# UVA-Computer-Vision-Lab/LabelAny3D

Hardware: AMD Instinct MI355X
Metric: fitted 3D boxes/sec @640x480 (higher is better)
Workload: dtype f64

## Files before the change

labelany3d_amd/csrc/la3d_device.hpp:

```cpp
#pragma once
#ifndef LA3D_NT
#define LA3D_NT 512
#endif
#include <hip/hip_runtime.h>
#include <mutex>
#include <utility>
#include <vector>
#include <math.h>
#include <stdint.h>
#include <stdio.h>
#include <string.h>

#include "la3d.h"

namespace la3d {


constexpr int NT = LA3D_NT;
constexpr int NWAVE = NT / 64;
constexpr int NTP = 256;
constexpr int NWAVEP = NTP / 64;
constexpr double PI_2 = 1.57079632679489661923;
typedef unsigned int u32x4 __attribute__((ext_vector_type(4)));

// ... 489 lines not shown
    for (int i = tid; i < nwords; i += NTH) {
      const unsigned w = src[i];
      bits[i] = w;
      n += __popc(w);
    }
  }
  if ((HW & 31) && tid == owner) {
    const unsigned w = bits[nwords - 1], keep = w & ((1u << (HW & 31)) - 1u);
    bits[nwords - 1] = keep;
    n -= __popc(w ^ keep);
  }
  return n;
}

constexpr int GEO_D = 20;

struct alignas(16) Shared {
  double part[NWAVE][7];
  double M[9];
  double Rg[9];
  double cyaw, syaw;
  int cnt[NWAVE];
  int nmask[NWAVE];
  unsigned scan[NWAVE];
  int n_valid;
  int st;
  int bad_ground;
  int redo;
  double gap;
  int nm;
  int order_inst;
  unsigned qhead;
  int sep_bad;
  unsigned qpad[2];
#ifdef LA3D_TIMELINE
  double* tl;
#endif
};
#ifndef LA3D_TIMELINE
static_assert(sizeof(Shared) == 752, "include/la3d.h (convex-hull yaw, rule 2) and oracle/campaigns/hull.py state this size");
#endif
__device__ inline void write_no_box(const FitParams& p, int inst, int status, double n_valid, double nm) {
  if (p.aux) {
    double* a = p.aux + (long long)inst * LA3D_AUX;
    a[0] = NAN; a[1] = n_valid; a[2] = nm; a[3] = NAN;
  }
  p.status[inst] = status;
  write_nan_box(p.out + (long long)inst * LA3D_REC);
  if (p.proj) { for (int j = 0; j < 8; ++j) p.proj[(long long)inst * 8 + j] = NAN; }
}
__device__ inline void write_no_box_axis(const Shared* sh, const FitParams& p, int inst) {
  if (p.aux) {
    double* a = p.aux + (long long)inst * LA3D_AUX;
    a[0] = atan2(sh->syaw, sh->cyaw); a[1] = (double)sh->n_valid; a[2] = (double)sh->nm; a[3] = sh->gap;
  }
  p.status[inst] = sh->st;
  write_nan_box(p.out + (long long)inst * LA3D_REC);
  if (p.proj) { for (int j = 0; j < 8; ++j) p.proj[(long long)inst * 8 + j] = NAN; }
}

#ifdef LA3D_TIMELINE
#define LA3D_SUBSTAMP(sh, k) do { if (threadIdx.x == 0 && (sh)->tl) (sh)->tl[k] = (double)wall_clock64(); } while (0)
#else
#define LA3D_SUBSTAMP(sh, k) do { } while (0)
#endif

__host__ __device__ inline int mask_bit_bytes(int HW) { return ((((HW + 15) / 16 + 1) / 2) * 4 + 15) & ~15; }
// ... 120 lines not shown
      } else {
        double x = d * r0, z = d * r2;
        if (PIV) { x = fma(d, r0, m ? -px0 : 0.0); z = fma(d, r2, m ? -pz0 : 0.0); }
        s[0] += x; s[1] += z;
        s[2] = fma(x, x, s[2]); s[3] = fma(x, z, s[3]); s[4] = fma(z, z, s[4]);
      }
      if (CHK) *n -= m;
    } else {
      const unsigned bits = db[k] | ~(unsigned)m;
      const double d = (double)__uint_as_float(bits);
      const double x = d * r0, z = d * r2;
      s[0] = dmin(s[0], x); s[1] = dmax(s[1], x);
      s[4] = dmin(s[4], z); s[5] = dmax(s[5], z);
      if (SPEC) {
        fk[k] = __uint_as_float(bits);
      } else {
        const double y = d * r1;
        s[2] = dmin(s[2], y); s[3] = dmax(s[3], y);
        r1 += a10;
      }
    }
    r0 += a00;
    if (!(SPEC && PASS == 0)) r2 += a20;
  }
  if (SPEC && PASS == 1) {
    const double dlo = (double)min_f32_raw(min3_f32(fk[0], fk[1], fk[2]), fk[3]);
    const double dhi = (double)max_f32_raw(max3_f32(fk[0], fk[1], fk[2]), fk[3]);
    const double ya = dlo * r1, yb = dhi * r1;
    s[2] = dmin(s[2], dmin(ya, yb)); s[3] = dmax(s[3], dmax(ya, yb));
  }
}


template <int NTH>
__device__ inline void column_xor_scan(unsigned* bits, int H, int ntx, unsigned* scratch, int scratch_words, int tid) {
  int RB = NTH / ntx;
  if (RB > scratch_words / ntx) RB = scratch_words / ntx;
  if (RB < 1) RB = 1;
  const int RPB = (H + RB - 1) / RB;
  const int items = ntx * RB;
  if (RB > 1) {
    for (int it = tid; it < items; it += NTH) {
      const int blk = it / ntx, cw = it - blk * ntx;
      const int r1 = min(blk * RPB + RPB, H);
      unsigned x = 0;
      for (int r = blk * RPB; r < r1; ++r) x ^= bits[r * ntx + cw];
      scratch[it] = x;
    }
    __syncthreads();
  }
  for (int it = tid; it < items; it += NTH) {
    const int blk = it / ntx, cw = it - blk * ntx;
    const int r1 = min(blk * RPB + RPB, H);
    unsigned carry = 0;
    for (int b2 = 0; b2 < blk; ++b2) carry ^= scratch[b2 * ntx + cw];
    for (int r = blk * RPB; r < r1; ++r) {
      carry ^= bits[r * ntx + cw];
      bits[r * ntx + cw] = carry;
    }
  }
}

template <int NTH>
__device__ inline int rle_to_bits(const int* __restrict__ counts, int nr, unsigned* bits, int nwords, int H, int W,
                                  unsigned* wtot, int tid, unsigned* scratch = nullptr, int scratch_words = 0, int frame_w = 0) {
  const int lane = tid & 63, wave = tid >> 6;
  constexpr int NW = NTH / 64;
  const int HW = H * (frame_w > 0 && frame_w < W ? frame_w : W);
  const float rcpH = 1.0f / (float)H;
  for (int i = tid; i < nwords; i += NTH) bits[i] = 0;
  unsigned carry = 0;
  int nm = 0;
  const bool toggles = (W & 31) == 0 && scratch != nullptr && scratch_words >= 2 * (W >> 5);
  for (int c0 = 0; c0 < nr; c0 += NTH) {
    const int j = c0 + tid;
    unsigned len = 0;
    if (j < nr) { const int v = counts[j]; len = v > 0 ? (unsigned)v : 0u; }
    unsigned incl = len;
#pragma unroll
    for (int o = 1; o < 64; o <<= 1) {
      const unsigned t = __shfl_up(incl, o);
      if (lane >= o) incl += t;
    }
    __syncthreads();
    if (lane == 63) wtot[wave] = incl;
    __syncthreads();
    unsigned base = carry, total = 0;
    for (int w = 0; w < NW; ++w) { if (w < wave) base += wtot[w]; total += wtot[w]; }
    const unsigned start = base + incl - len;
    unsigned L = 0;
    if ((j & 1) && len > 0 && start < (unsigned)HW) L = min(len, (unsigned)HW - start);
    nm += (int)L;
    carry += total;
    unsigned long long todo = __ballot(L != 0);
    if (toggles) {
      const int ntx = W >> 5;
      unsigned long long wrap = 0;
      unsigned c_first = 0, c_last = 0;
      if (L != 0) {
        unsigned col0, row0, cole, rowe;
        pix_uv(start, H, rcpH, &row0, &col0);
        pix_uv(start + L, H, rcpH, &rowe, &cole);
        atomicXor(&bits[row0 * ntx + (col0 >> 5)], 1u << (col0 & 31));
        if (rowe != 0) atomicXor(&bits[rowe * ntx + (cole >> 5)], 1u << (cole & 31));
        c_first = col0 + 1;
        c_last = rowe != 0 ? cole : cole - 1;
      }
      wrap = __ballot(L != 0 && c_last >= c_first);
      while (wrap) {
        const int src = __ffsll((long long)wrap) - 1;
        wrap &= wrap - 1;
        const unsigned cf = (unsigned)__builtin_amdgcn_readlane((int)c_first, src);
        const unsigned cl = (unsigned)__builtin_amdgcn_readlane((int)c_last, src);
        for (unsigned cw = (cf >> 5) + lane; cw <= (cl >> 5); cw += 64) {
          const unsigned lo = cw == (cf >> 5) ? (cf & 31u) : 0u, hi = cw == (cl >> 5) ? (cl & 31u) : 31u;
          atomicXor(&bits[cw], (0xffffffffu >> (31u - hi)) & (0xffffffffu << lo));
        }
      }
      todo = 0;
    }
    while (todo) {
      const int src = __ffsll((long long)todo) - 1;
      todo &= todo - 1;
      const unsigned S = __shfl(start, src), Lr = __shfl(L, src);
      unsigned col0, row0;
      pix_uv(S, H, rcpH, &row0, &col0);
      if (row0 + Lr <= (unsigned)H) {
        const unsigned base = row0 * (unsigned)W + col0;
        for (unsigned q = lane; q < Lr; q += 64) {
          const unsigned idx = base + q * (unsigned)W;
          atomicOr(&bits[idx >> 5], 1u << (idx & 31));
        }
      } else {
        for (unsigned q = lane; q < Lr; q += 64) {
          unsigned col, row;
          pix_uv(S + q, H, rcpH, &row, &col);
          const unsigned idx = row * (unsigned)W + col;
          atomicOr(&bits[idx >> 5], 1u << (idx & 31));
        }
      }
    }
    if (carry >= (unsigned)HW) break;
  }
  __syncthreads();
  if (toggles) {
    column_xor_scan<NTH>(bits, H, W >> 5, scratch, scratch_words, tid);
    __syncthreads();
  }
  return nm;
}

inline int check_launch(const char* what) {
  const hipError_t e = hipGetLastError();
  if (e != hipSuccess) {
    snprintf(g_err, sizeof(g_err), "%s: %s", what, hipGetErrorString(e));
    return LA3D_ERR_HIP;
  }
  return LA3D_SUCCESS;
}

inline void allow_big_lds(const void* fn, int bytes = 160 * 1024) {
  static std::mutex mu;
  static std::vector<std::pair<const void*, int>> done;
  int dev = 0;
  if (hipGetDevice(&dev) != hipSuccess) (void)hipGetLastError();
  std::lock_guard<std::mutex> g(mu);
  for (const auto& d : done)
    if (d.first == fn && d.second == dev) return;
  if (hipFuncSetAttribute(fn, hipFuncAttributeMaxDynamicSharedMemorySize, bytes) != hipSuccess) (void)hipGetLastError();
  done.emplace_back(fn, dev);
}

constexpr int CULL_MIN = 224;
constexpr int MAX_MASK_LDS = 128 * 1024;

}
```

labelany3d_amd/csrc/la3d_instance.hip:

```cpp
#include <algorithm>
#include <atomic>
#include <chrono>
#include <cstdint>
#include <cstddef>
#include <cstring>
#include <mutex>
#include <type_traits>
#include <utility>
#include <vector>

#include "la3d_device.hpp"
#include "la3d_poly.hpp"
#include "la3d_engines.hpp"
#include "la3d_walks.hpp"
#include "la3d_stages.hpp"
#include "la3d_instance_phases.hpp"
#include "la3d_hull.hpp"

#ifndef LA3D_INSTANCE_DT
#define LA3D_INSTANCE_DT 0
#endif
#if LA3D_INSTANCE_DT == 0
using DepthT = float;
using KParams = la3d::FitParams;
// ... 170 lines not shown
    while (wall_clock64() - t0 < w) __builtin_amdgcn_s_sleep(32);
  }
  int my_draw = 0;
  if (SAMPLE && tid < LA3D_NSAMPLE) my_draw = p.sample_idx[(long long)inst * LA3D_NSAMPLE + tid];
  int nmask = 0;
  if constexpr (LDSMASK) nmask = mask_to_bits<VEC, SRC, FRAMES>(p, p_call, inst, mpl, bits, sh, list, TILED ? p.list_cap / 2 : 0, tid, wave, lane);
  __syncthreads();
  LA3D_STAMP(1);
  const int inst_p = __builtin_amdgcn_readfirstlane(sh->order_inst);
  if constexpr (FRAMES) frame_geometry<false, SAMPLE>(p_frame, p_call, p.image_index[inst_p]);
  const int tid_plain = tid;
#define tid (REBUILD_TID ? tid_here(wave, lane) : tid_plain)
  if (SRC != 0 && LDSMASK && p.filter_boundary >= 0) {
    if (!filter_keep<SRC>(p, sh, bits, inst_p, tid)) return;
  }
  double Mg[9];
#pragma unroll
  for (int i = 0; i < 9; ++i) Mg[i] = uniform_f64(sh->M[i]);
  LA3D_STAMP(13);

  bool sampled = false;
  int ntot = 0;
  if (SAMPLE) {
    const int wsum = wave_sum_i(nmask);
    if (lane == 0) sh->nmask[wave] = wsum;
    __syncthreads();
    for (int w = 0; w < NWAVE; ++w) ntot += sh->nmask[w];
    sampled = HULL || ntot > LA3D_NSAMPLE;
  }

  constexpr bool LK = TILED && !SAMPLE;
  const bool sep_cam = LK && (HULL || !p.sep_off) && Mg[1] == 0.0 && Mg[3] == 0.0 && Mg[6] == 0.0 && Mg[7] == 0.0 && Mg[8] == 1.0;
  TileList tiles;
  if (TILED && !sampled) {
    if constexpr (FRAMES) frame_rcp_ntx(p_frame);
    tiles = build_tile_list<LK>(p, sh, bits, list, sep_cam, tid, wave, lane);
    LA3D_STAMP(15);
    __syncthreads();
  }
  const int nactive = tiles.nactive, nfull = tiles.nfull, compact = tiles.compact;
  const bool sep = tiles.sep;

  if constexpr (HULL && LK) {
    hull_full_mask(sh, p, inst_p, dpl, bits, list, nactive, sep, Mg, nmask, wave, lane, cv);
    return;
  }

  if constexpr (LK) {
    if (sep) {
      LA3D_STAMP(2);
      unsigned* col = bits + nactive * 8;
      double sacc[5] = {0, 0, 0, 0, 0}, yx[2] = {INFINITY, -INFINITY};
      unsigned unsafe = 0u;
      if (p.H & 7) sweep_sep<true>(p, dpl, bits, list, nactive, Mg, col, wave, lane, sacc, yx, &unsafe, 0, nfull, cv);
      else sweep_sep<false>(p, dpl, bits, list, nactive, Mg, col, wave, lane, sacc, yx, &unsafe, 0, nfull, cv);
      if (__ballot(unsafe >= 0x7f800000u) != 0ull && lane == 0) sh->sep_bad = 1;
      const double ylo_w = uniform_f64(wave_min(yx[0])), yhi_w = uniform_f64(wave_max(yx[1]));
      LA3D_STAMP(3);
      stage_moments_to_axis(sh, p, inst_p, sacc, nmask, nmask, tid, wave, lane, true);
      LA3D_STAMP(4);
      if (!(sh->redo || sh->sep_bad)) {
        if (sh->st != LA3D_BOX_OK) return;
        double N0[3], N2[3], ext[6];
        yaw_rows(sh, Mg, N0, N2);
        sep_col_extents(col, p.W, N0, N2, tid, ext);
        ext[2] = ylo_w; ext[3] = yhi_w;
        LA3D_STAMP(5);
        if constexpr (FRAMES) frame_proj(p_frame, p_call, inst_p);
        stage_extents_to_box(sh, p, inst_p, ext, tid, wave, lane);
        stage_status_aux(sh, p, inst_p, tid);
        LA3D_STAMP(6);
        return;
      }
      __syncthreads();
    }
  }

  bool cull = false;
  int rng_words = 0;
  if constexpr (LK) {
    if (compact) {
      rng_words = cull_rng_words(nactive);
      cull = nactive >= p.cull_min && nactive <= CULL_MAXT;
      if (!cull) {
        unsigned short* surv = reinterpret_cast<unsigned short*>(bits + nactive * 8);
#pragma clang loop vectorize(disable) interleave(disable) unroll(disable)
        for (int t = tid; t < nactive; t += NT) surv[t] = (unsigned short)t;
      }
    }
  }

  LA3D_STAMP(2);
  double acc[5] = {0, 0, 0, 0, 0};
  int cnt = 0;
  double px = 0, py = 0, pz = 0;
  bool pok = false;

  if (SAMPLE) {
// ... 248 lines not shown
```

labelany3d_amd/csrc/la3d_instance_phases.hpp:

```cpp
#pragma once
#include "la3d_device.hpp"
#include "la3d_poly.hpp"
#include "la3d_hull.hpp"

using namespace la3d;

namespace {
template <bool VEC, int SRC, bool FRAMES>
__device__ inline int mask_to_bits(const FitParams& p, const FitParams& call, int inst, const unsigned char* mpl, unsigned* bits, Shared* sh,
                                   void* stage, int stage_words, int tid, int wave, int lane) {
  const int HW = p.HW;
  int nmask = 0;
  if constexpr (SRC == 1) {
    const long long o0 = p.rle_offsets[inst];
    nmask = rle_to_bits<NT>(p.rle_counts + o0, (int)(p.rle_offsets[inst + 1] - o0), bits, p.nwords, p.H, p.W, sh->scan, tid,
                            static_cast<unsigned*>(stage), stage_words, p.frame_w);
  } else if constexpr (SRC == 2) {
    nmask = poly_to_bits<NT>(p.poly_xy, p.poly_ring_off, p.poly_inst_rings[inst], p.poly_inst_rings[inst + 1],
                             static_cast<PolySide*>(stage), sh->scan, bits, p.nwords, p.H, p.W, tid, p.frame_w);
  } else if constexpr (SRC == 3) {
    if constexpr (FRAMES) nmask = bits_plane_to_lds<NT>(p.mask_bits + frame_bits_offset(call, inst), bits, p.nwords, HW, 1, tid);
    else nmask = bits_plane_to_lds<NT>(p.mask_bits + (long long)inst * p.bits_plane_stride, bits, p.nwords, HW, p.bits_vec, tid);
  } else {
    unsigned short* b16 = reinterpret_cast<unsigned short*>(bits);
    const int ngroups = (HW + 15) >> 4;
    if (VEC) {
      const u32x4* m4 = reinterpret_cast<const u32x4*>(mpl);
      constexpr int P0U = 4;
      unsigned seen = 0;
#pragma unroll P0U
      for (int g = tid; g < ngroups; g += NT) {
        const u32x4 w = __builtin_nontemporal_load(m4 + g);
        const unsigned lo = __builtin_amdgcn_udot4(w.y, 0x80402010u, __builtin_amdgcn_udot4(w.x, 0x08040201u, 0u, false), false);
        const unsigned hi = __builtin_amdgcn_udot4(w.w, 0x80402010u, __builtin_amdgcn_udot4(w.z, 0x08040201u, 0u, false), false);
        const unsigned pat = lo | (hi << 8);
        seen |= (w.x | w.y) | (w.z | w.w);
        b16[g] = (unsigned short)pat;
        nmask += __popc(pat);
      }
      const unsigned long long odd = __ballot((seen & 0xfefefefeu) != 0);
      if (lane == 0) sh->scan[wave] = odd != 0 ? 1u : 0u;
      __syncthreads();
      unsigned general = 0;
#pragma unroll
      for (int w = 0; w < NWAVE; ++w) general |= sh->scan[w];
      if (general) {
        nmask = 0;
#pragma unroll 4
        for (int g = tid; g < ngroups; g += NT) {
          const u32x4 w = m4[g];
          const unsigned pat = nz16(w.x, w.y, w.z, w.w);
          b16[g] = (unsigned short)pat;
// ... 1 lines not shown
        }
      }
    } else {
      for (int g = tid; g < ngroups; g += NT) {
        unsigned pat = 0;
        for (int k = 0; k < 16; ++k) {
          const int i = g * 16 + k;
          if (i < HW && mpl[i]) pat |= 1u << k;
        }
        b16[g] = (unsigned short)pat;
        nmask += __popc(pat);
      }
    }
    if ((ngroups & 1) && tid == 0) b16[ngroups] = 0;
  }
  return nmask;
}

template <int SRC>
__device__ inline bool filter_keep(const FitParams& p, Shared* sh, const unsigned* bits, int inst, int tid) {
  int st4[4];
  bits_filter_stats<NT>(bits, p.H, p.frame_w, p.filter_boundary, reinterpret_cast<int*>(sh->part), tid, st4, p.W);
  if (p.filter_stats && tid < 4) (p.filter_stats + (long long)inst * 4)[tid] = st4[tid];
  const int height = SRC == 1 ? st4[1] : (SRC == 3 && !p.bits_span) ? st4[1] : st4[2];
  const bool keep = 16 * height > p.H && st4[3] < p.filter_max_edge && st4[0] >= p.filter_min_area;
  if (!keep && tid == 0) write_no_box(p, inst, LA3D_BOX_FILTERED, 0.0, (double)st4[0]);
  return keep;
}

struct TileList {
  int nactive = 0, nfull = 0, compact = 0;
  bool sep = false;
};

template <bool WHOLE_ROWS, bool LK>
__device__ inline void classify_tiles(const FitParams& p, const unsigned* bits, int tbeg, int tend, int lane, unsigned long long* bal,
                                      unsigned (*wrd)[8], int* wcount, int* fcount, unsigned* fl) {
#pragma unroll
  for (int k = 0; k < 4; ++k) {
    const int t = tbeg + k * 64 + lane;
    unsigned any = 0, all = 0xffffffffu;
    if (t < tend) {
      const int ty = (int)(((float)t + 0.5f) * p.rcp_ntx), tx = t - ty * p.ntx;
      const int rmax = p.H - 1 - ty * 8;
      const unsigned* bw = bits + (ty * 8) * p.ntx + tx;
#pragma unroll
      for (int rr = 0; rr < 8; ++rr) {
        const unsigned w = bw[(WHOLE_ROWS ? rr : min(rr, rmax)) * p.ntx];
        any |= w;
        if constexpr (LK) { wrd[k][rr] = (WHOLE_ROWS || rr <= rmax) ? w : 0u; all &= wrd[k][rr]; }
      }
    }
    bal[k] = __ballot(any != 0);
    *wcount += __popcll(bal[k]);
    if constexpr (LK) {
      const bool f = t < tend && all == 0xffffffffu;
      *fcount += __popcll(__ballot(f));
      *fl |= (f ? 1u : 0u) << k;
    }
  }
}

template <bool LK>
__device__ inline TileList build_tile_list(const FitParams& p, Shared* sh, unsigned* bits, unsigned short* list, bool sep_cam, int tid, int wave, int lane) {
  TileList tl;
  const int ntiles = p.ntx * p.nty, per = p.tiles_per_wave;
// ... 51 lines not shown
  } else {
#pragma unroll 1
    for (int pass = 0; pass < 2; ++pass) {
      int wcount = 0;
      for (int t0 = tbeg; t0 < tend; t0 += 64) {
        const int t = t0 + lane;
        unsigned any = 0, packed = 0;
        if (t < tend) {
          const int ty = t / p.ntx, tx = t - ty * p.ntx;
          const int rows = min(8, p.H - ty * 8);
          const unsigned* bw = bits + (ty * 8) * p.ntx + tx;
          for (int rr = 0; rr < rows; ++rr) any |= bw[rr * p.ntx];
          packed = ((unsigned)ty << 8) | (unsigned)tx;
        }
        const unsigned long long bal = __ballot(any != 0);
        if (pass == 1 && any) list[base + wcount + __popcll(bal & ((1ull << lane) - 1ull))] = (unsigned short)packed;
        wcount += __popcll(bal);
      }
      if (pass == 0) {
        if (lane == 0) sh->scan[wave] = (unsigned)wcount;
        __syncthreads();
        for (int w = 0; w < NWAVE; ++w) {
          const int c = (int)sh->scan[w];
          if (w < wave) base += c;
          tl.nactive += c;
        }
        if (tl.nactive > p.list_cap) { tl.nactive = -1; break; }
      }
    }
  }
  return tl;
}

template <bool HULL, bool FRAMES, typename DepthT>
__device__ inline void sample_pick(const FitParams& p, Shared* sh, const unsigned* bits, unsigned* prefix, const DepthT* __restrict__ dpl,
                                          const DepthCvt<DepthT> cv, const double* Mg, int ntot, int my_draw, int tid, int wave, int lane,
                                          double* acc, int* cnt, double* ppx, double* ppy, double* ppz, bool* ppok) {
  const int nblk = (p.nwords + 31) >> 5;
  unsigned run0 = 0;
  for (int b0 = 0; b0 < nblk; b0 += NT) {
    const int blk = b0 + tid;
    unsigned local = 0;
    if (blk < nblk) {
      const int w0 = blk << 5, wn = min(32, p.nwords - w0);
      if (wn == 32) {
        const uint4* q = reinterpret_cast<const uint4*>(bits + w0);
#pragma unroll
        for (int i = 0; i < 8; ++i) { const uint4 v = q[i]; local += __popc(v.x) + __popc(v.y) + __popc(v.z) + __popc(v.w); }
      } else {
        for (int i = 0; i < wn; ++i) local += __popc(bits[w0 + i]);
      }
    }
    unsigned incl = local;
#pragma unroll
    for (int o = 1; o < 64; o <<= 1) {
      const unsigned t = __shfl_up(incl, o);
      if (lane >= o) incl += t;
    }
    if (lane == 63) sh->scan[wave] = incl;
    __syncthreads();
    unsigned base = run0, tot = 0;
    for (int w = 0; w < NWAVE; ++w) { const unsigned c = sh->scan[w]; if (w < wave) base += c; tot += c; }
    if (blk < nblk) prefix[blk] = base + incl - local;
    run0 += tot;
    __syncthreads();
  }
// ... 64 lines not shown
```

labelany3d_amd/csrc/la3d_poly.hpp:

```cpp
#pragma once
#include "la3d_device.hpp"

namespace la3d {

struct alignas(8) PolyEdge {
  int y0, y1;
  long long x, dx;
};

struct alignas(8) PolySide {
  PolyEdge e;
  int sx, sy, ex, ey;
};

constexpr int POLY_XY_SHIFT = 16;
constexpr int POLY_CHUNK = 32;
constexpr int POLY_MAX_JOINT = 8;
constexpr int POLY_META_INTS = 48;
constexpr int POLY_STAGE_BYTES = POLY_CHUNK * (int)sizeof(PolySide) + POLY_META_INTS * 4;
#ifndef LA3D_POLY_KEEP
#define LA3D_POLY_KEEP 4
#endif
constexpr int POLY_KEEP = LA3D_POLY_KEEP;

// ... 78 lines not shown

__device__ inline void poly_set_bit(unsigned* bits, int W, int x, int y) {
  const unsigned i = (unsigned)y * (unsigned)W + (unsigned)x;
  atomicOr(&bits[i >> 5], 1u << (i & 31));
}

__device__ inline void poly_draw(const PolySide& s, int W, unsigned* bits, int lane) {
  if (s.sx > s.ex) return;
  const int dx = s.ex - s.sx, dy = s.ey - s.sy;
  const int ady = dy < 0 ? -dy : dy, sgn = dy < 0 ? -1 : 1;
  if (ady > dx) {
    for (int i = lane; i <= ady; i += 64) {
      const int k = (int)((2u * (unsigned)i * (unsigned)dx + (unsigned)ady - 1u) / (2u * (unsigned)ady));
      poly_set_bit(bits, W, s.sx + k, s.sy + sgn * i);
    }
  } else {
    for (int i = lane; i <= dx; i += 64) {
      const int k = dx ? (int)((2u * (unsigned)i * (unsigned)ady + (unsigned)dx - 1u) / (2u * (unsigned)dx)) : 0;
      poly_set_bit(bits, W, s.sx + i, s.sy + sgn * k);
    }
  }
}

__device__ inline void poly_fill_span(unsigned* bits, int W, int y, int x1, int x2) {
  const unsigned i1 = (unsigned)y * (unsigned)W + (unsigned)x1, i2 = (unsigned)y * (unsigned)W + (unsigned)x2;
  const unsigned w1 = i1 >> 5, w2 = i2 >> 5;
  const unsigned m1 = 0xffffffffu << (i1 & 31), m2 = 0xffffffffu >> (31 - (i2 & 31));
  if (w1 == w2) { atomicOr(&bits[w1], m1 & m2); return; }
  atomicOr(&bits[w1], m1);
  for (unsigned w = w1 + 1; w < w2; ++w) atomicOr(&bits[w], 0xffffffffu);
  atomicOr(&bits[w2], m2);
}

template <int NTH>
__device__ __forceinline__ void poly_ring_fast(const int* __restrict__ xy, long long p0, int n, const int* rb, int nrb, PolySide* stage,
                                      int* box, unsigned* bits, int H, int W, int tid, int clipW) {
  const int lane = tid & 63, wave = tid >> 6;
  constexpr int NW = NTH / 64;
  const int ntxw = W >> 5;
  if (tid == 0) { box[0] = H; box[1] = 0; box[2] = ntxw; box[3] = 0; }
  for (int pass = 0; pass < 2; ++pass) {
    for (int c0 = 0; c0 < n; c0 += POLY_CHUNK) {
      const int m = min(POLY_CHUNK, n - c0);
      if (pass == 0 || n > POLY_CHUNK) {
        __syncthreads();
        if (tid < m) {
          const int i = c0 + tid;
          int lo = 0, hi = n;
          for (int j = 0; j < nrb; ++j)
            if (i >= rb[j] && i < rb[j + 1]) { lo = rb[j]; hi = rb[j + 1]; }
          const int ip = (i == lo) ? hi - 1 : i - 1;
          const PolySide sd = poly_side(xy[2 * (p0 + ip)], xy[2 * (p0 + ip) + 1], xy[2 * (p0 + i)], xy[2 * (p0 + i) + 1], clipW, H);
          stage[tid] = sd;
          if (pass == 0 && sd.e.y0 < sd.e.y1) {
            const int ya = max(sd.e.y0, 0), yb = min(sd.e.y1, H);
            if (ya < yb) {
              const long long fa = (sd.e.x + (long long)(ya - sd.e.y0) * sd.e.dx) >> POLY_XY_SHIFT;
              const long long fb = (sd.e.x + (long long)(yb - 1 - sd.e.y0) * sd.e.dx) >> POLY_XY_SHIFT;
              const long long lo = (fa < fb ? fa : fb) + 1, hi = (fa < fb ? fb : fa) + 1;
              atomicMin(&box[0], ya); atomicMax(&box[1], yb);
              if (lo < W) atomicMin(&box[2], (int)((lo < 0 ? 0 : lo) >> 5));
              atomicMax(&box[3], (int)((hi >= W ? W - 1 : (hi < 0 ? 0 : hi)) >> 5));
            }
          }
        }
      }
      __syncthreads();
      for (int j = wave; j < m; j += NW) {
        if (pass == 1) poly_draw(stage[j], W, bits, lane);
        const int y0 = stage[j].e.y0, y1 = stage[j].e.y1;
        if (y0 >= y1) continue;
        const long long ex = stage[j].e.x, edx = stage[j].e.dx;
        const int yb = min(y1, H);
        for (int y = max(y0, 0) + lane; y < yb; y += 64) {
          const long long f = (ex + (long long)(y - y0) * edx) >> POLY_XY_SHIFT;
          if (pass == 0) {
            const long long pos = f < -1 ? 0 : f + 1;
            if (pos < W) atomicXor(&bits[y * ntxw + (int)(pos >> 5)], 1u << ((int)pos & 31));
          } else if (f >= 0 && f < W) {
            atomicOr(&bits[y * ntxw + (int)(f >> 5)], 1u << ((int)f & 31));
          }
        }
      }
    }
    if (pass == 0) {
// ... 63 lines not shown
                }
              }
            }
          }
        }
      }
      const int npairs = min(found, POLY_KEEP) >> 1;
#pragma unroll
      for (int k = 0; k < POLY_KEEP / 2; ++k) {
        if (k < npairs) {
          const long long c1 = cx[2 * k] >> POLY_XY_SHIFT, c2 = cx[2 * k + 1] >> POLY_XY_SHIFT;
          if (c1 < W && c2 >= 0) poly_fill_span(bits, W, y, (int)(c1 < 0 ? 0 : c1), (int)(c2 >= W ? W - 1 : c2));
        }
      }
      const bool more = found > POLY_KEEP;
      if (more) { lastx = cx[POLY_KEEP - 1]; lasti = ci[POLY_KEEP - 1]; }
      first = false;
      const unsigned long long any = __ballot(more);
      __syncthreads();
      if (lane == 0) flags[wave] = any != 0 ? 1u : 0u;
      __syncthreads();
      unsigned again = 0;
#pragma unroll
      for (int w = 0; w < NW; ++w) again |= flags[w];
      if (!again) break;
    }
  }
}

__device__ inline long long poly_uniform(long long v) {
  return ((long long)__builtin_amdgcn_readfirstlane((int)(v >> 32)) << 32) | (unsigned)__builtin_amdgcn_readfirstlane((int)v);
}

template <int NTH>
__device__ __forceinline__ int poly_to_bits(const int* __restrict__ xy, const long long* __restrict__ ring_off, long long r0, long long r1,
                                   PolySide* stage, unsigned* flags, unsigned* bits, int nwords, int H, int W, int tid, int clipW = 0) {
  if (clipW <= 0 || clipW > W) clipW = W;
  r0 = poly_uniform(r0); r1 = poly_uniform(r1);
  for (int i = tid; i < nwords; i += NTH) bits[i] = 0;
  int* meta = reinterpret_cast<int*>(stage + POLY_CHUNK);
  const int nr = (int)(r1 - r0);
  long long r = r0;
  if (nr >= 1 && (W & 31) == 0) {
    int joint = 1;
    if (nr >= 2 && nr <= POLY_MAX_JOINT) {
      const int lane = tid & 63, wave = tid >> 6;
      const long long pf = ring_off[r0];
      for (int j = wave; j < nr; j += NTH / 64) {
        const long long a = ring_off[r0 + j], b = ring_off[r0 + j + 1];
        int x0 = 0x7fffffff, x1 = -0x7fffffff - 1, y0 = 0x7fffffff, y1 = -0x7fffffff - 1;
        for (long long q = a + lane; q < b; q += 64) {
          const int x = xy[2 * q], y = xy[2 * q + 1];
          x0 = min(x0, x); x1 = max(x1, x); y0 = min(y0, y); y1 = max(y1, y);
        }
        x0 = wave_min_i(x0); x1 = wave_max_i(x1); y0 = wave_min_i(y0); y1 = wave_max_i(y1);
        if (lane == 0) { meta[9 + 4 * j] = x0; meta[10 + 4 * j] = x1; meta[11 + 4 * j] = y0; meta[12 + 4 * j] = y1; meta[j] = (int)(a - pf); }
      }
      if (tid == 0) meta[nr] = (int)(ring_off[r1] - pf);
      __syncthreads();
      if (tid == 0) {
        int ok = 1;
        for (int i = 0; i < nr; ++i)
          for (int j = i + 1; j < nr; ++j) {
            const bool apart = meta[10 + 4 * i] < meta[9 + 4 * j] || meta[10 + 4 * j] < meta[9 + 4 * i] ||
                               meta[12 + 4 * i] < meta[11 + 4 * j] || meta[12 + 4 * j] < meta[11 + 4 * i];
            if (!apart) ok = 0;
          }
        meta[41] = ok;
      }
      __syncthreads();
      if (meta[41]) joint = nr;
    }
    const long long p0 = poly_uniform(ring_off[r0]);
    const int n = __builtin_amdgcn_readfirstlane((int)(ring_off[r0 + joint] - p0));
    if (joint == 1) {
      if (tid == 0) { meta[0] = 0; meta[1] = n; }
      __syncthreads();
    }
    poly_ring_fast<NTH>(xy, p0, n, meta, joint, stage, reinterpret_cast<int*>(flags), bits, H, W, tid, clipW);
    r = r0 + joint;
  }
  for (; r < r1; ++r) {
    const long long p0 = poly_uniform(ring_off[r]);
    const int n = __builtin_amdgcn_readfirstlane((int)(ring_off[r + 1] - p0));
    poly_ring_general<NTH>(xy, p0, n, stage, flags, bits, H, W, tid, clipW);
  }
  __syncthreads();
  if (clipW < W) {
    const int ntxw = W >> 5, wq = clipW >> 5, per = ntxw - wq;
    const unsigned keep = (1u << (clipW & 31)) - 1u;
    for (int i = tid; i < H * per; i += NTH) {
      const int row = i / per, k = i - row * per;
      unsigned* w = bits + row * ntxw + wq + k;
      *w = k == 0 ? (*w & keep) : 0u;
    }
    __syncthreads();
  }
  int nm = 0;
  for (int i = tid; i < nwords; i += NTH) nm += __popc(bits[i]);
  return nm;
}

__device__ inline void bits_stats_256(const unsigned* bits, int H, int W, int boundary, int* rowcnt, int* red, int tid, int* out4) {
  const int lane = tid & 63, wave = tid >> 6;
  const int bc = min(boundary, W), br = min(boundary, H);
  int area = 0, edge = 0;
  for (int r = tid; r < H; r += 256) {
    int cnt = 0, e = 0;
    const unsigned base = (unsigned)r * (unsigned)W;
    for (int c0 = 0; c0 < W; c0 += 32) {
      const unsigned i = base + c0, wi = i >> 5, sh = i & 31;
      unsigned w = bits[wi] >> sh;
      if (sh && c0 + (32 - (int)sh) < W) w |= bits[wi + 1] << (32 - sh);
      const int valid = min(32, W - c0);
      if (valid < 32) w &= (1u << valid) - 1u;
      cnt += __popc(w);
      const int nlo = min(max(bc - c0, 0), 32), fhi = min(max(W - bc - c0, 0), 32);
      e += __popc(nlo >= 32 ? w : (w & ((1u << nlo) - 1u))) + __popc(fhi >= 32 ? 0u : (w & ~((1u << fhi) - 1u)));
    }
    rowcnt[r] = cnt;
    area += cnt;
    edge += e + cnt * ((r < br ? 1 : 0) + (r >= H - br ? 1 : 0));
  }
  area = wave_sum_i(area);
  edge = wave_sum_i(edge);
  if (lane == 0) { red[12 + wave] = area; red[16 + wave] = edge; }
  __syncthreads();
  int rows = 0, first = H, last = -1;
  for (int r = tid; r < H; r += 256)
    if (rowcnt[r] != 0) { rows += 1; first = min(first, r); last = max(last, r); }
  rows = wave_sum_i(rows);
// ... 13 lines not shown
```

labelany3d_amd/csrc/la3d_walks.hpp:

```cpp
#pragma once
#include "la3d_device.hpp"

using namespace la3d;

namespace {
template <bool VEC, bool LDSMASK, int PASS, bool PIV = false, typename DT = float>
__device__ inline void sweep(const FitParams& p, const DT* __restrict__ dpl, const unsigned char* __restrict__ mpl,
                             const unsigned* bits, const double* A0, const double* A1, const double* A2,
                             int wave, int lane, double* acc, int* cnt, int* nmask, const double* pivot = nullptr,
                             const DepthCvt<DT> cv = {}) {
  double px0 = 0, pz0 = 0;
  if constexpr (PIV) { px0 = pivot[0]; pz0 = pivot[1]; }
  const int HW = p.HW, W = p.W;
  const int nquads = (HW + 3) >> 2;
  const int nchunks = (nquads + 63) >> 6;
  const double a00 = A0[0], a01 = A0[1], a02 = A0[2];
  const double a20 = A2[0], a21 = A2[1], a22 = A2[2];
  double a10 = 0, a11 = 0, a12 = 0;
  if (PASS == 1) { a10 = A1[0]; a11 = A1[1]; a12 = A1[2]; }
  double s0 = acc[0], s1 = acc[1], s2 = acc[2], s3 = acc[3], s4 = acc[4];
  double xlo = acc[0], xhi = acc[1], ylo = acc[2], yhi = acc[3], zlo = acc[4], zhi = acc[5];
  int n = *cnt, nm = *nmask;
  for (int ch = wave; ch < nchunks; ch += NWAVE) {
    const int q = ch * 64 + lane;
// ... 405 lines not shown
        ry += a11;
      }
      const double r0 = fma(a00, (double)(tx * 32 + c), a02);
      const double t1 = r0 * c1, t2 = r0 * c2;
      s0 += t1; s1 += c1; s2 = fma(r0, t2, s2); s3 += t2; s4 += c2;
      bad = max(bad, cmax);
      atomicMin(colq + tx * 32, cmin);
      atomicMax(colq + tx * 32 + p.W, cmax);
      __builtin_amdgcn_sched_barrier(0);
    }
  }
}

template <bool EDGE = false, typename DT = float>
__device__ inline void sweep_sep(const FitParams& p, const DT* __restrict__ dpl, const unsigned* bits,
                                 const unsigned short* list, int nactive, const double* Mg, unsigned* col, int wave, int lane,
                                 double* acc, double* yext, unsigned* unsafe, int row0 = 0, int nfull = 0, const DepthCvt<DT> cv = {}) {
  const int c = lane & 31, h4 = (lane >> 5) * 4;
  const double a00 = Mg[0], a02 = Mg[2], a11 = Mg[4], a12 = Mg[5];
  unsigned loff[4];
#pragma unroll
  for (int k = 0; k < 4; ++k) loff[k] = (unsigned)((h4 + k) * p.W + c) * (unsigned)sizeof(DT);
  unsigned* colq = col + c;
  double s0 = acc[0], s1 = acc[1], s2 = acc[2], s3 = acc[3], s4 = acc[4];
  double ylo = yext[0], yhi = yext[1];
  unsigned bad = *unsafe;
  if (nfull > 0) sep_steps<EDGE, true, DT>(p, dpl, bits, list, 0, nfull, a00, a02, a11, a12, colq, wave, c, h4, loff, row0, s0, s1, s2, s3, s4, ylo, yhi, bad, cv);
  sep_steps<EDGE, false, DT>(p, dpl, bits, list, nfull, nactive, a00, a02, a11, a12, colq, wave, c, h4, loff, row0, s0, s1, s2, s3, s4, ylo, yhi, bad, cv);
  acc[0] = s0; acc[1] = s1; acc[2] = s2; acc[3] = s3; acc[4] = s4;
  yext[0] = ylo; yext[1] = yhi;
  *unsafe = bad;
}

__device__ inline void sep_col_extents(const unsigned* col, int W, const double* N0, const double* N2, int tid, double* ext) {
  double xlo = INFINITY, xhi = -INFINITY, zlo = INFINITY, zhi = -INFINITY;
  for (int u = tid; u < W; u += NT) {
    const unsigned lo = col[u], hi = col[W + u];
    if (lo <= hi) {
      const double dlo = (double)__uint_as_float(lo), dhi = (double)__uint_as_float(hi), ud = (double)u;
      const double q0 = fma(N0[0], ud, N0[2]), q2 = fma(N2[0], ud, N2[2]);
      const double xa = dlo * q0, xb = dhi * q0, za = dlo * q2, zb = dhi * q2;
      xlo = fmin(xlo, fmin(xa, xb)); xhi = fmax(xhi, fmax(xa, xb));
      zlo = fmin(zlo, fmin(za, zb)); zhi = fmax(zhi, fmax(za, zb));
    }
  }
  ext[0] = xlo; ext[1] = xhi; ext[4] = zlo; ext[5] = zhi;
}

}
```

Measured before the change: 11.72 million.

## Track mask bounding box during decode and restrict scan, tiling, and extents to it

RLE and polygon decoders now record a coarse bounding box of the mask (in 32-column words and 8-row tiles) and pack it into shared memory. The column XOR scan, popcount, tile classification/list build, and column-extent reduction then iterate only over that box instead of the full frame. This targets work spent on empty regions of small masks. In exchange it adds atomics for box tracking, a fallback to the full frame when the box logic does not apply, and edge-case risk in box clipping.

```diff
diff --git a/labelany3d_amd/csrc/la3d_device.hpp b/labelany3d_amd/csrc/la3d_device.hpp
--- a/labelany3d_amd/csrc/la3d_device.hpp
+++ b/labelany3d_amd/csrc/la3d_device.hpp
@@ -545,7 +545,8 @@
   int order_inst;
   unsigned qhead;
   int sep_bad;
-  unsigned qpad[2];
+  unsigned mbox;
+  unsigned qpad;
 #ifdef LA3D_TIMELINE
   double* tl;
 #endif
@@ -732,6 +733,49 @@
 }
 
 
+constexpr unsigned MASK_BOX_EMPTY = 0x00010001u;
+__device__ inline unsigned mask_box_pack(int c0, int c1, int r0, int r1) {
+  if (c1 < c0 || r1 < r0) return MASK_BOX_EMPTY;
+  return (unsigned)min(c0 >> 5, 255) | ((unsigned)min(c1 >> 5, 255) << 8) | ((unsigned)min(r0 >> 3, 255) << 16) | ((unsigned)min(r1 >> 3, 255) << 24);
+}
+__device__ inline unsigned mask_box_whole(int H, int W) { return mask_box_pack(0, W - 1, 0, H - 1); }
+
+template <int NTH>
+__device__ inline void column_xor_scan(unsigned* bits, int H, int ntx, unsigned* scratch, int scratch_words, int tid);
+
+template <int NTH>
+__device__ inline void column_xor_scan_box(unsigned* bits, int H, int ntx, int cw0, int ncw, int r0, int nrows, unsigned* scratch,
+                                           int scratch_words, int tid) {
+  if (ncw > NTH || ncw > scratch_words) {
+    column_xor_scan<NTH>(bits, H, ntx, scratch, scratch_words, tid);
+    return;
+  }
+  const float rcp = 1.0f / (float)ncw;
+  int RB = (int)(((float)min(NTH, scratch_words) + 0.5f) * rcp);
+  RB = max(min(min(RB, 24), nrows), 1);
+  const int RPB = (int)(((float)(nrows + RB - 1) + 0.5f) * (1.0f / (float)RB));
+  const int items = ncw * RB;
+  const int blk = (int)(((float)tid + 0.5f) * rcp), c = tid - blk * ncw;
+  const int ra = r0 + blk * RPB, rb = min(ra + RPB, r0 + nrows);
+  unsigned* bw = bits + cw0 + c;
+  if (RB > 1) {
+    if (tid < items) {
+      unsigned x = 0;
+      for (int r = ra; r < rb; ++r) x ^= bw[r * ntx];
+      scratch[tid] = x;
+    }
+    __syncthreads();
+  }
+  if (tid < items) {
+    unsigned carry = 0;
+    for (int b2 = 0; b2 < blk; ++b2) carry ^= scratch[b2 * ncw + c];
+    for (int r = ra; r < rb; ++r) {
+      carry ^= bw[r * ntx];
+      bw[r * ntx] = carry;
+    }
+  }
+}
+
 template <int NTH>
 __device__ inline void column_xor_scan(unsigned* bits, int H, int ntx, unsigned* scratch, int scratch_words, int tid) {
   int RB = NTH / ntx;
@@ -761,9 +805,10 @@
   }
 }
 
-template <int NTH>
+template <int NTH, bool BOX = false>
 __device__ inline int rle_to_bits(const int* __restrict__ counts, int nr, unsigned* bits, int nwords, int H, int W,
-                                  unsigned* wtot, int tid, unsigned* scratch = nullptr, int scratch_words = 0, int frame_w = 0) {
+                                  unsigned* wtot, int tid, unsigned* scratch = nullptr, int scratch_words = 0, int frame_w = 0,
+                                  unsigned* box_out = nullptr) {
   const int lane = tid & 63, wave = tid >> 6;
   constexpr int NW = NTH / 64;
   const int HW = H * (frame_w > 0 && frame_w < W ? frame_w : W);
@@ -772,6 +817,12 @@
   unsigned carry = 0;
   int nm = 0;
   const bool toggles = (W & 31) == 0 && scratch != nullptr && scratch_words >= 2 * (W >> 5);
+  const bool boxed = BOX && toggles && scratch_words >= 2 * (W >> 5) + 4;
+  int* gbox = reinterpret_cast<int*>(scratch + (boxed ? scratch_words - 4 : 0));
+  int bc0 = 0x7fffffff, bc1 = -1, br0 = 0x7fffffff, br1 = -1;
+  if constexpr (BOX) {
+    if (boxed && tid == 0) { gbox[0] = 0x7fffffff; gbox[1] = -1; gbox[2] = 0x7fffffff; gbox[3] = -1; }
+  }
   for (int c0 = 0; c0 < nr; c0 += NTH) {
     const int j = c0 + tid;
     unsigned len = 0;
@@ -805,6 +856,12 @@
         if (rowe != 0) atomicXor(&bits[rowe * ntx + (cole >> 5)], 1u << (cole & 31));
         c_first = col0 + 1;
         c_last = rowe != 0 ? cole : cole - 1;
+        if constexpr (BOX) {
+          bc0 = min(bc0, (int)col0); bc1 = max(bc1, (int)c_last);
+          const bool one_col = c_last == col0;
+          br0 = one_col ? min(br0, (int)row0) : 0;
+          br1 = one_col ? max(br1, rowe != 0 ? (int)rowe - 1 : H - 1) : H - 1;
+        }
       }
       wrap = __ballot(L != 0 && c_last >= c_first);
       while (wrap) {
@@ -842,7 +899,24 @@
     }
     if (carry >= (unsigned)HW) break;
   }
+  if constexpr (BOX) {
+    if (boxed) {
+      bc0 = wave_min_i(bc0); bc1 = wave_max_i(bc1); br0 = wave_min_i(br0); br1 = wave_max_i(br1);
+      if (lane == 0 && bc1 >= 0) { atomicMin(&gbox[0], bc0); atomicMax(&gbox[1], bc1); atomicMin(&gbox[2], br0); atomicMax(&gbox[3], br1); }
+    }
+  }
   __syncthreads();
+  if constexpr (BOX) {
+    if (boxed) {
+      const int c0 = __builtin_amdgcn_readfirstlane(gbox[0]), c1 = __builtin_amdgcn_readfirstlane(gbox[1]);
+      const int r0 = __builtin_amdgcn_readfirstlane(gbox[2]), r1 = __builtin_amdgcn_readfirstlane(gbox[3]);
+      if (c1 >= c0) column_xor_scan_box<NTH>(bits, H, W >> 5, c0 >> 5, (c1 >> 5) - (c0 >> 5) + 1, r0, min(r1 + 1, H - 1) - r0 + 1, scratch, scratch_words - 4, tid);
+      if (tid == 0) *box_out = mask_box_pack(c0, c1, r0, r1);
+      __syncthreads();
+      return nm;
+    }
+    if (tid == 0) *box_out = mask_box_whole(H, W);
+  }
   if (toggles) {
     column_xor_scan<NTH>(bits, H, W >> 5, scratch, scratch_words, tid);
     __syncthreads();
diff --git a/labelany3d_amd/csrc/la3d_instance.hip b/labelany3d_amd/csrc/la3d_instance.hip
--- a/labelany3d_amd/csrc/la3d_instance.hip
+++ b/labelany3d_amd/csrc/la3d_instance.hip
@@ -226,9 +226,17 @@
   constexpr bool LK = TILED && !SAMPLE;
   const bool sep_cam = LK && (HULL || !p.sep_off) && Mg[1] == 0.0 && Mg[3] == 0.0 && Mg[6] == 0.0 && Mg[7] == 0.0 && Mg[8] == 1.0;
   TileList tiles;
+  constexpr bool BOXED = TILED && (SRC == 1 || SRC == 2);
+  struct NoBox {};
+  std::conditional_t<BOXED, TileBox, NoBox> tbox;
   if (TILED && !sampled) {
     if constexpr (FRAMES) frame_rcp_ntx(p_frame);
-    tiles = build_tile_list<LK>(p, sh, bits, list, sep_cam, tid, wave, lane);
+    if constexpr (BOXED) {
+      tbox = tile_box_load(sh, p.W, !HULL);
+      tiles = build_tile_list_box<LK>(p, sh, bits, list, sep_cam, tid, wave, lane, tbox);
+    } else {
+      tiles = build_tile_list<LK>(p, sh, bits, list, sep_cam, tid, wave, lane);
+    }
     LA3D_STAMP(15);
     __syncthreads();
   }
@@ -257,7 +265,8 @@
         if (sh->st != LA3D_BOX_OK) return;
         double N0[3], N2[3], ext[6];
         yaw_rows(sh, Mg, N0, N2);
-        sep_col_extents(col, p.W, N0, N2, tid, ext);
+        if constexpr (BOXED) sep_col_extents<true>(col, p.W, N0, N2, tid, ext, tbox.u0, tbox.u1);
+        else sep_col_extents(col, p.W, N0, N2, tid, ext);
         ext[2] = ylo_w; ext[3] = yhi_w;
         LA3D_STAMP(5);
         if constexpr (FRAMES) frame_proj(p_frame, p_call, inst_p);
diff --git a/labelany3d_amd/csrc/la3d_instance_phases.hpp b/labelany3d_amd/csrc/la3d_instance_phases.hpp
--- a/labelany3d_amd/csrc/la3d_instance_phases.hpp
+++ b/labelany3d_amd/csrc/la3d_instance_phases.hpp
@@ -13,11 +13,11 @@
   int nmask = 0;
   if constexpr (SRC == 1) {
     const long long o0 = p.rle_offsets[inst];
-    nmask = rle_to_bits<NT>(p.rle_counts + o0, (int)(p.rle_offsets[inst + 1] - o0), bits, p.nwords, p.H, p.W, sh->scan, tid,
-                            static_cast<unsigned*>(stage), stage_words, p.frame_w);
+    nmask = rle_to_bits<NT, true>(p.rle_counts + o0, (int)(p.rle_offsets[inst + 1] - o0), bits, p.nwords, p.H, p.W, sh->scan, tid,
+                                  static_cast<unsigned*>(stage), stage_words, p.frame_w, &sh->mbox);
   } else if constexpr (SRC == 2) {
-    nmask = poly_to_bits<NT>(p.poly_xy, p.poly_ring_off, p.poly_inst_rings[inst], p.poly_inst_rings[inst + 1],
-                             static_cast<PolySide*>(stage), sh->scan, bits, p.nwords, p.H, p.W, tid, p.frame_w);
+    nmask = poly_to_bits<NT, true>(p.poly_xy, p.poly_ring_off, p.poly_inst_rings[inst], p.poly_inst_rings[inst + 1],
+                                   static_cast<PolySide*>(stage), sh->scan, bits, p.nwords, p.H, p.W, tid, p.frame_w, &sh->mbox);
   } else if constexpr (SRC == 3) {
     if constexpr (FRAMES) nmask = bits_plane_to_lds<NT>(p.mask_bits + frame_bits_offset(call, inst), bits, p.nwords, HW, 1, tid);
     else nmask = bits_plane_to_lds<NT>(p.mask_bits + (long long)inst * p.bits_plane_stride, bits, p.nwords, HW, p.bits_vec, tid);
@@ -85,6 +85,19 @@
   int nactive = 0, nfull = 0, compact = 0;
   bool sep = false;
 };
+
+struct TileBox {
+  int tx0 = 0, ty0 = 0, bw = 0, bh = 0, u0 = 0, u1 = 0;
+};
+__device__ inline TileBox tile_box_load(const Shared* sh, int W, bool cols) {
+  const unsigned m = (unsigned)__builtin_amdgcn_readfirstlane((int)sh->mbox);
+  TileBox b;
+  b.tx0 = (int)(m & 0xffu); b.ty0 = (int)((m >> 16) & 0xffu);
+  b.bw = max((int)((m >> 8) & 0xffu) - b.tx0 + 1, 0); b.bh = max((int)(m >> 24) - b.ty0 + 1, 0);
+  if (b.bw == 0 || b.bh == 0) b.bw = b.bh = 0;
+  b.u0 = cols ? b.tx0 * 32 : 0; b.u1 = cols ? (b.tx0 + b.bw) * 32 : W;
+  return b;
+}
 
 template <bool WHOLE_ROWS, bool LK>
 __device__ inline void classify_tiles(const FitParams& p, const unsigned* bits, int tbeg, int tend, int lane, unsigned long long* bal,
@@ -202,6 +215,96 @@
   return tl;
 }
 
+template <bool WHOLE_ROWS, bool LK>
+__device__ inline void classify_tiles_box(const FitParams& p, const unsigned* bits, int tbeg, int tend, int lane, unsigned long long* bal,
+                                          unsigned (*wrd)[8], int* wcount, int* fcount, unsigned* fl, const TileBox& box, float rcp_bw, int per) {
+#pragma unroll
+  for (int k = 0; k < 4; ++k) {
+    if (k * 64 >= per) { bal[k] = 0ull; continue; }
+    const int t = tbeg + k * 64 + lane;
+    unsigned any = 0, all = 0xffffffffu;
+    if (t < tend) {
+      const int by = (int)(((float)t + 0.5f) * rcp_bw), ty = box.ty0 + by, tx = box.tx0 + t - by * box.bw;
+      const int rmax = p.H - 1 - ty * 8;
+      const unsigned* bw = bits + (ty * 8) * p.ntx + tx;
+#pragma unroll
+      for (int rr = 0; rr < 8; ++rr) {
+        const unsigned w = bw[(WHOLE_ROWS ? rr : min(rr, rmax)) * p.ntx];
+        any |= w;
+        if constexpr (LK) { wrd[k][rr] = (WHOLE_ROWS || rr <= rmax) ? w : 0u; all &= wrd[k][rr]; }
+      }
+    }
+    bal[k] = __ballot(any != 0);
+    *wcount += __popcll(bal[k]);
+    if constexpr (LK) {
+      const bool f = t < tend && all == 0xffffffffu;
+      *fcount += __popcll(__ballot(f));
+      *fl |= (f ? 1u : 0u) << k;
+    }
+  }
+}
+
+template <bool LK>
+__device__ inline TileList build_tile_list_box(const FitParams& p, Shared* sh, unsigned* bits, unsigned short* list, bool sep_cam, int tid, int wave, int lane,
+                                               const TileBox& box) {
+  if (p.tiles_per_wave > 256) return build_tile_list<LK>(p, sh, bits, list, sep_cam, tid, wave, lane);
+  TileList tl;
+  const int ntiles = box.bw * box.bh, per = (ntiles + NWAVE - 1) / NWAVE;
+  const int tbeg = wave * per, tend = min(tbeg + per, ntiles);
+  const float rcp_bw = __int_as_float(__builtin_amdgcn_readfirstlane(__float_as_int(1.0f / (float)max(box.bw, 1))));
+  int base = 0;
+  unsigned long long bal[4];
+  unsigned wrd[LK ? 4 : 1][8];
+  int wcount = 0, fcount = 0;
+  unsigned fl = 0;
+  if ((p.H & 7) == 0) classify_tiles_box<true, LK>(p, bits, tbeg, tend, lane, bal, wrd, &wcount, &fcount, &fl, box, rcp_bw, per);
+  else classify_tiles_box<false, LK>(p, bits, tbeg, tend, lane, bal, wrd, &wcount, &fcount, &fl, box, rcp_bw, per);
+  if (lane == 0) sh->scan[wave] = (unsigned)wcount | ((unsigned)fcount << 16);
+  __syncthreads();
+  LA3D_SUBSTAMP(sh, 14);
+  int fbase = 0;
+  for (int w = 0; w < NWAVE; ++w) {
+    const int c = (int)(sh->scan[w] & 0xffffu), f = (int)(sh->scan[w] >> 16);
+    if (w < wave) { base += c - f; fbase += f; }
+    tl.nactive += c;
+    tl.nfull += f;
+  }
+  if (tl.nactive > p.list_cap) {
+    tl.nactive = -1;
+    tl.nfull = 0;
+    return tl;
+  }
+  if constexpr (LK) tl.compact = (tl.nactive * 32 + cull_rng_words(tl.nactive) * 4 <= p.mask_lds_bytes) ? 1 : 0;
+  int foff = fbase, poff = tl.nfull + base;
+#pragma unroll
+  for (int k = 0; k < 4; ++k) {
+    if (k * 64 >= per) continue;
+    const bool isf = LK && ((fl >> k) & 1u);
+    const unsigned long long bf = LK ? __ballot(isf) : 0ull, bp = bal[k] & ~bf, lt = (1ull << lane) - 1ull;
+    if ((bal[k] >> lane) & 1ull) {
+      const int t = tbeg + k * 64 + lane;
+      const int by = (int)(((float)t + 0.5f) * rcp_bw), ty = box.ty0 + by, tx = box.tx0 + t - by * box.bw;
+      const int idx = isf ? foff + __popcll(bf & lt) : poff + __popcll(bp & lt);
+      list[idx] = (unsigned short)((ty << 8) | tx);
+      if constexpr (LK) if (tl.compact) {
+        uint4* e = reinterpret_cast<uint4*>(bits) + 2 * idx;
+        e[0] = make_uint4(wrd[k][0], wrd[k][1], wrd[k][2], wrd[k][3]);
+        e[1] = make_uint4(wrd[k][4], wrd[k][5], wrd[k][6], wrd[k][7]);
+      }
+    }
+    foff += __popcll(bf); poff += __popcll(bp);
+  }
+  if constexpr (LK) if (tl.compact) {
+    if (sep_cam && tl.nactive * 32 + sep_col_words(p.W) * 4 <= p.mask_lds_bytes) {
+      tl.sep = true;
+      unsigned* col = bits + tl.nactive * 8;
+#pragma clang loop vectorize(disable) interleave(disable) unroll(disable)
+      for (int u = box.u0 + tid; u < box.u1; u += NT) { col[u] = 0xffffffffu; col[p.W + u] = 0u; }
+    }
+  }
+  return tl;
+}
+
 template <bool HULL, bool FRAMES, typename DepthT>
 __device__ inline void sample_pick(const FitParams& p, Shared* sh, const unsigned* bits, unsigned* prefix, const DepthT* __restrict__ dpl,
                                           const DepthCvt<DepthT> cv, const double* Mg, int ntot, int my_draw, int tid, int wave, int lane,
diff --git a/labelany3d_amd/csrc/la3d_poly.hpp b/labelany3d_amd/csrc/la3d_poly.hpp
--- a/labelany3d_amd/csrc/la3d_poly.hpp
+++ b/labelany3d_amd/csrc/la3d_poly.hpp
@@ -134,13 +134,17 @@
   atomicOr(&bits[w2], m2);
 }
 
-template <int NTH>
+template <int NTH, bool BOX = false>
 __device__ __forceinline__ void poly_ring_fast(const int* __restrict__ xy, long long p0, int n, const int* rb, int nrb, PolySide* stage,
                                       int* box, unsigned* bits, int H, int W, int tid, int clipW) {
   const int lane = tid & 63, wave = tid >> 6;
   constexpr int NW = NTH / 64;
   const int ntxw = W >> 5;
   if (tid == 0) { box[0] = H; box[1] = 0; box[2] = ntxw; box[3] = 0; }
+  if constexpr (BOX) {
+    static_assert(!BOX || NTH >= 512, "the vertex box lives in flags[4..7]");
+    if (tid == 0) { box[4] = 0x7fffffff; box[5] = -0x7fffffff - 1; box[6] = 0x7fffffff; box[7] = -0x7fffffff - 1; }
+  }
   for (int pass = 0; pass < 2; ++pass) {
     for (int c0 = 0; c0 < n; c0 += POLY_CHUNK) {
       const int m = min(POLY_CHUNK, n - c0);
@@ -152,7 +156,16 @@
           for (int j = 0; j < nrb; ++j)
             if (i >= rb[j] && i < rb[j + 1]) { lo = rb[j]; hi = rb[j + 1]; }
           const int ip = (i == lo) ? hi - 1 : i - 1;
-          const PolySide sd = poly_side(xy[2 * (p0 + ip)], xy[2 * (p0 + ip) + 1], xy[2 * (p0 + i)], xy[2 * (p0 + i) + 1], clipW, H);
+          PolySide sd;
+          if constexpr (BOX) {
+            const int vx = xy[2 * (p0 + i)], vy = xy[2 * (p0 + i) + 1];
+            sd = poly_side(xy[2 * (p0 + ip)], xy[2 * (p0 + ip) + 1], vx, vy, clipW, H);
+            if (pass == 0) {
+              atomicMin(&box[4], vx); atomicMax(&box[5], vx); atomicMin(&box[6], vy); atomicMax(&box[7], vy);
+            }
+          } else {
+            sd = poly_side(xy[2 * (p0 + ip)], xy[2 * (p0 + ip) + 1], xy[2 * (p0 + i)], xy[2 * (p0 + i) + 1], clipW, H);
+          }
           stage[tid] = sd;
           if (pass == 0 && sd.e.y0 < sd.e.y1) {
             const int ya = max(sd.e.y0, 0), yb = min(sd.e.y1, H);
@@ -282,15 +295,18 @@
   return ((long long)__builtin_amdgcn_readfirstlane((int)(v >> 32)) << 32) | (unsigned)__builtin_amdgcn_readfirstlane((int)v);
 }
 
-template <int NTH>
+template <int NTH, bool BOX = false>
 __device__ __forceinline__ int poly_to_bits(const int* __restrict__ xy, const long long* __restrict__ ring_off, long long r0, long long r1,
-                                   PolySide* stage, unsigned* flags, unsigned* bits, int nwords, int H, int W, int tid, int clipW = 0) {
+                                   PolySide* stage, unsigned* flags, unsigned* bits, int nwords, int H, int W, int tid, int clipW = 0,
+                                   unsigned* box_out = nullptr) {
   if (clipW <= 0 || clipW > W) clipW = W;
   r0 = poly_uniform(r0); r1 = poly_uniform(r1);
   for (int i = tid; i < nwords; i += NTH) bits[i] = 0;
   int* meta = reinterpret_cast<int*>(stage + POLY_CHUNK);
   const int nr = (int)(r1 - r0);
   long long r = r0;
+  int vx0 = 0, vx1 = 0, vy0 = 0, vy1 = 0;
+  bool whole = true;
   if (nr >= 1 && (W & 31) == 0) {
     int joint = 1;
     if (nr >= 2 && nr <= POLY_MAX_JOINT) {
@@ -327,8 +343,14 @@
       if (tid == 0) { meta[0] = 0; meta[1] = n; }
       __syncthreads();
     }
-    poly_ring_fast<NTH>(xy, p0, n, meta, joint, stage, reinterpret_cast<int*>(flags), bits, H, W, tid, clipW);
+    poly_ring_fast<NTH, BOX>(xy, p0, n, meta, joint, stage, reinterpret_cast<int*>(flags), bits, H, W, tid, clipW);
     r = r0 + joint;
+    if constexpr (BOX) {
+      const int* vb = reinterpret_cast<const int*>(flags) + 4;
+      vx0 = __builtin_amdgcn_readfirstlane(vb[0]); vx1 = __builtin_amdgcn_readfirstlane(vb[1]);
+      vy0 = __builtin_amdgcn_readfirstlane(vb[2]); vy1 = __builtin_amdgcn_readfirstlane(vb[3]);
+      whole = r < r1;
+    }
   }
   for (; r < r1; ++r) {
     const long long p0 = poly_uniform(ring_off[r]);
@@ -347,6 +369,22 @@
     __syncthreads();
   }
   int nm = 0;
+  if constexpr (BOX) {
+    if (!whole) {
+      const int c0 = max(vx0, 1) - 1, c1 = min(vx1, clipW - 2) + 1, q0 = max(vy0, 1) - 1, q1 = min(vy1, H - 2) + 1;
+      if (tid == 0) *box_out = mask_box_pack(c0, c1, q0, q1);
+      if (c0 <= c1 && q0 <= q1) {
+        const int ntxw = W >> 5, end = (q1 + 1) * ntxw;
+        for (int i = q0 * ntxw + tid; i < end; i += 4 * NTH) {
+          const unsigned a = bits[i], b = i + NTH < end ? bits[i + NTH] : 0u, c = i + 2 * NTH < end ? bits[i + 2 * NTH] : 0u,
+                         d = i + 3 * NTH < end ? bits[i + 3 * NTH] : 0u;
+          nm += __popc(a) + __popc(b) + __popc(c) + __popc(d);
+        }
+      }
+      return nm;
+    }
+    if (tid == 0) *box_out = mask_box_whole(H, W);
+  }
   for (int i = tid; i < nwords; i += NTH) nm += __popc(bits[i]);
   return nm;
 }
diff --git a/labelany3d_amd/csrc/la3d_walks.hpp b/labelany3d_amd/csrc/la3d_walks.hpp
--- a/labelany3d_amd/csrc/la3d_walks.hpp
+++ b/labelany3d_amd/csrc/la3d_walks.hpp
@@ -461,9 +461,10 @@
   *unsafe = bad;
 }
 
-__device__ inline void sep_col_extents(const unsigned* col, int W, const double* N0, const double* N2, int tid, double* ext) {
+template <bool BOX = false>
+__device__ inline void sep_col_extents(const unsigned* col, int W, const double* N0, const double* N2, int tid, double* ext, int u0 = 0, int u1 = 0) {
   double xlo = INFINITY, xhi = -INFINITY, zlo = INFINITY, zhi = -INFINITY;
-  for (int u = tid; u < W; u += NT) {
+  for (int u = (BOX ? u0 : 0) + tid; u < (BOX ? u1 : W); u += NT) {
     const unsigned lo = col[u], hi = col[W + u];
     if (lo <= hi) {
       const double dlo = (double)__uint_as_float(lo), dhi = (double)__uint_as_float(hi), ud = (double)u;
diff --git a/profiles/annot_box/summarize_annot_box.py b/profiles/annot_box/summarize_annot_box.py
--- /dev/null
+++ b/profiles/annot_box/summarize_annot_box.py
@@ -0,0 +1,58 @@
+import collections
+import csv
+import glob
+import json
+import os
+import re
+import statistics
+import sys
+
+
+def bench_line(path):
+    for line in open(path):
+        line = line.strip()
+        if line.startswith("{"):
+            return json.loads(line)
+    return None
+
+
+def table(out):
+    runs = collections.defaultdict(lambda: {"launch": [], "step": []})
+    for f in sorted(glob.glob(os.path.join(out, "*.json"))):
+        m = re.match(r"(parent|branch)_(.+)_(\d+)\.json$", os.path.basename(f))
+        j = bench_line(f) if m else None
+        if j is None:
+            continue
+        runs[(m.group(2), m.group(1))]["launch"].append(j["roofline"]["avg_launch_ms"] * 1e3)
+        runs[(m.group(2), m.group(1))]["step"].append(j["ms_per_step"] * 1e3)
+    fmt = lambda v: f"{statistics.median(v):.2f} ({min(v):.2f} - {max(v):.2f})"
+    print("| line | runs | parent avg_launch µs | branch avg_launch µs | parent ms_per_step µs | branch ms_per_step µs | ranges apart |")
+    print("|---|---|---|---|---|---|---|")
+    for tag in sorted({k[0] for k in runs}):
+        p, b = runs[(tag, "parent")], runs[(tag, "branch")]
+        apart = "yes" if max(b["launch"]) < min(p["launch"]) and max(b["step"]) < min(p["step"]) else "no"
+        print(f"| {tag} | {len(p['launch'])} | {fmt(p['launch'])} | {fmt(b['launch'])} | {fmt(p['step'])} | {fmt(b['step'])} | {apart} |")
+
+
+def counters(d, tree, kind):
+    for f in glob.glob(d + "/sq/**/*counter_collection.csv", recursive=True):
+        acc, n = collections.defaultdict(lambda: collections.defaultdict(float)), collections.Counter()
+        for r in csv.DictReader(open(f)):
+            kn = r["Kernel_Name"]
+            if "fit_instances" not in kn:
+                continue
+            acc[kn][r["Counter_Name"]] += float(r["Counter_Value"])
+            n[kn] += r["Counter_Name"] == "SQ_INSTS_VALU"
+        for kn in acc:
+            print(tree, kind, kn[:90], "launches", n[kn], {c: round(v / n[kn]) for c, v in acc[kn].items()})
+    for f in glob.glob(d + "/stats/**/*kernel_stats.csv", recursive=True):
+        for r in csv.DictReader(open(f)):
+            if "fit_instances" in r["Name"]:
+                print(tree, kind, "stats", r["Name"][:90], "calls", r["Calls"], "avg_ns", r["AverageNs"], "min", r["MinNs"], "max", r["MaxNs"])
+
+
+if __name__ == "__main__":
+    if sys.argv[1] == "table":
+        table(sys.argv[2])
+    else:
+        counters(*sys.argv[2:5])
```

Result: no change. 11.63 million (-0.8%).
